# tub-rip/event_based_bos

Hardware: AMD Instinct MI355X
Metric: Mevents/sec warped+IWE at 1280x720 (higher is better)
Workload: dtype f32

## Files before the change

event_based_bos_amd/_hip.py:

```python
from __future__ import annotations

import ctypes as C
import os
from typing import Optional

import torch

_PKG_DIR = os.path.dirname(os.path.abspath(__file__))
LIB_PATH = os.path.join(_PKG_DIR, "lib", "libebos_hip.so")

EBOS_OK = 0
REF_FIRST, REF_LAST, REF_FRACTION, REF_TIMEBASE = 0, 1, 2, 3
SPLAT_BILINEAR, SPLAT_COUNT, SPLAT_POLARITY = 0, 1, 2
GAUSS_REFLECT_SCIPY, GAUSS_REFLECT_TORCH = 0, 1
PROFILE_SLAB_ACCUMULATE, PROFILE_TILED_BWD, PROFILE_SLAB_COMBINE, PROFILE_GRADMAG_FUSED = 0, 1, 2, 3
ABI_VERSION = 2
GML_NO_POLARITY, GML_EVENT_WEIGHTS = 1, 2
GML_VELOCITY = 4



_HW_QUEUES = 4
MAX_HW_QUEUES = 2

# ... 81 lines not shown
    "ebos_raw_time_range": (_I, [_P, _I, _L, _D, _P, _P, _P]),
    "ebos_raw_events_to_soa": (_I, [_P, _P, _P, _I, _P, _D, _P, _I, _D, _I, _L, _P, _P, _P, _P, _P]),
    "ebos_bin_scratch_bytes": (_Z, [_L]),
    "ebos_bin_scratch_bytes_events": (_Z, [_L, _I, _I, _I, _I]),
    "ebos_bin_events_f32": (_I, [_P, _P, _P, _P, _L, _I, _I, _I, _I, _P, _P, _P, _P, _P, _P, _P, _P, _P, _Z, _P]),
    "ebos_plan_lean_scratch_bytes": (_Z, [_L, _I, _I, _I, _I]),
    "ebos_plan_lean": (_I, [_I, _P, _P, _P, _P, _D, _L, _I, _D, _I, _I, _I, _I, _I, _P, _P, _P, _P, _L, _P, _P, _P, _Z, _P]),
    "ebos_plan_compact_f32": (_I, [_P, _P, _P, _P, _L, _I, _I, _I, _I, _P, _P, _P, _L, _P]),
    "ebos_plan_compact_frac_f32": (_I, [_P, _P, _P, _P, _L, _I, _I, _I, _I, _P, _P, _P, _P, _P, _L, _P]),
    "ebos_iwe_dense_f32": (_I, [_P, _P, _P, _P, _L, _P, _I, _I, _I, _I, _I, _P, _P]),
    "ebos_iwe_dense_tiled_f32": (_I, [_P, _P, _P, _P, _P, _L, _P, _I, _I, _I, _I, _I, _I, _I, _I, _P, _P]),
    "ebos_tiled_config": (_I, [C.POINTER(C.c_int), _I]),
    "ebos_iwe_dense_bwd_f32": (_I, [_P, _P, _P, _P, _L, _P, _I, _I, _I, _I, _I, _P, _P, _I, _I, _P, _P, _P]),
    "ebos_slab_config": (_I, [C.POINTER(C.c_int), _I]),
    "ebos_halo_auto": (_I, [_I, _D]),
    "ebos_iwe_slab_workspace_bytes": (_Z, [_I, _I, _I, _I, _I, _I, _I, _I]),
    "ebos_iwe_dense_slab_f32": (_I, [_P, _P, _P, _P, _P, _P, _P, _P, _L, _P, _I, _I, _I, _I, _I, _I, _I, _I, _P, _Z, _P, _I, _I, _P, _P, _P, _P]),
    "ebos_iwe_2dof_slab_f32": (_I, [_P, _P, _P, _P, _P, _P, _P, _P, _L, _P, _I, _I, _I, _I, _I, _I, _I, _I, _I, _P, _Z, _P, _I, _I, _P, _P, _P, _P]),
    "ebos_iwe_2dof_slab_batch_f32": (_I, [_P, _P, _P, _P, _L, _P, _I, _I, _I, _I, _I, _I, _I, _I, _I, _P, _Z, _P, _I, _I, _P, _P, _P, _P, _P]),
    "ebos_plan_parts": (_I, [_P, _I, _I, _I, _I, _I, _I, _P, _P]),
    "ebos_plan_facts": (_I, [_P, _I, _I, _I, _I, _P, _P, _P, _P]),
    "ebos_iwe_2dof_tiled_bwd_f32": (_I, [_P, _P, _P, _P, _P, _P, _P, _P, _L, _P, _I, _I, _I, _I, _I, _I, _I, _I, _P, _P, _I, _P, _P, _Z, _P]),
    "ebos_iwe_dense_tiled_bwd_f32": (_I, [_P, _P, _P, _P, _P, _P, _P, _P, _L, _P, _I, _I, _I, _I, _I, _I, _I, _P, _P, _I, _P, _P, _P, _P, _P, _P, _Z, _P, _P]),
    "ebos_variance_dense_job_f32": (_I, [_P, _P, _P, _P, _P, _P]),
    "ebos_gradient_magnitude_dense_job_f32": (_I, [_P, _P, _P, _P, _P, _P, _P, _P, _L, _P]),
    "ebos_variance_dense_job_signed_f32": (_I, [_P, _P, _P, _P, _P, _P, _P]),
    "ebos_gradient_magnitude_fused_partials": (_L, [_I, _I]),
    "ebos_gradient_magnitude_fused_f32": (_I, [_P, _I, _I, _I, _P, _P, _P, _P, _L, _P]),
    "ebos_iwe_2dof_f32": (_I, [_P, _P, _P, _P, _L, _P, _I, _I, _I, _I, _I, _P, _P]),
    "ebos_iwe_2dof_bwd_f32": (_I, [_P, _P, _P, _P, _L, _P, _I, _I, _I, _I, _I, _P, _P, _I, _P, _P]),
# ... 246 lines not shown
```

event_based_bos_amd/csrc/iwe_tile_core.h:

```cpp
#pragma once
#include <stdlib.h>

#include <atomic>
#include <type_traits>

#include <hip/hip_ext.h>

#include "common.h"
#include "patch_grid.h"
#include "blur3.h"

namespace ebos {
namespace {

constexpr float kEps = 1e-6f;
constexpr int kBlock = 1024;

#ifdef EBOS_STAMPS
__device__ unsigned long long g_stamps[4096 * 8];
__device__ unsigned long long g_stamps_bwd[4096 * 8];
#define EBOS_STAMP(k)                                                                   \
  do {                                                                                  \
    if (threadIdx.x == 0 && blockIdx.x < 4096) g_stamps[blockIdx.x * 8 + (k)] = wall_clock64(); \
  } while (0)
// ... 377 lines not shown
}
__device__ __forceinline__ float slab_load1(__amdgpu_buffer_rsrc_t r, unsigned byte) {
  return __uint_as_float(__builtin_amdgcn_raw_buffer_load_b32(r, (int)byte, 0, kAuxSc1));
}
#endif

struct ChunkQueue {
  unsigned* next;
  __device__ __forceinline__ int pull() const {
    unsigned c = 0;
    if ((threadIdx.x & (kWave - 1)) == 0) c = atomicAdd(next, 1u);
    return (int)__builtin_amdgcn_readfirstlane(c);
  }
};

#ifdef EBOS_ABL_MULTIK
#define EBOS_KLOOP for (int kk = 0; kk < EBOS_ABL_MULTIK; ++kk)
#define EBOS_KOFF(v, s) ((v) + (s) * (float)kk)
#else
#define EBOS_KLOOP
#define EBOS_KOFF(v, s) (v)
#endif

__device__ __forceinline__ int32_t chunk_group(int32_t g_first, int c, int lane) { return g_first + c * kWave + lane; }

template <int TH, int TW, int HALO, bool UNIFORM, int MODE = ACC_FX, bool GRID = false, bool DYN = false, bool PAIRS = false,
          bool HAS_W = false>
__device__ __forceinline__ unsigned long long accumulate_compact_fx(const TileRange& tr, double* s_acc, const EvPtrs& ev,
                                                          const float* __restrict__ flow, int H, int W, bool* any_spill,
                                                          const ChunkQueue& queue, const Win<TH, TW, HALO, DYN>& win,
                                                          const CRaw* pre = nullptr, float wscale = kFxScale) {
  static_assert(!HAS_W || (MODE == ACC_FX && !PAIRS && !DYN), "per-event weights: the plain fixed-point loop on the largest window");
  constexpr bool kMerge = PAIRS && MODE == ACC_FX;
  const int LH = win.LH(), LW = win.LW(), HR = win.HR(), HC = win.HC(), PT = win.P();
  const unsigned kPlane = LH * PT / 2;
  const unsigned kDummy = LH * PT;
  constexpr float kMagic = 12582912.0f;
  constexpr int kMagicBits = 0x4B400000;
  const float* __restrict__ flow1 = UNIFORM ? flow : flow + (GRID ? (int64_t)TH * TW : (int64_t)H * W);
  const float uni_u = UNIFORM ? -flow[0] : 0.0f, uni_v = UNIFORM ? -flow[1] : 0.0f;
  const unsigned base_lin = GRID ? 0u : (unsigned)(tr.ty * TH * W + tr.tx * TW);
  const unsigned uW = GRID ? (unsigned)TW : (unsigned)W;
  constexpr bool kBuf = !UNIFORM && !GRID;
  const __amdgpu_buffer_rsrc_t rsrc = __builtin_amdgcn_make_buffer_rsrc(
      reinterpret_cast<char*>(const_cast<float*>(flow)) - 4 * HC, 0, kBuf ? 2 * H * W * (int)sizeof(float) + 4 * HC : 0, 0x00020000);
  const int soff0 = (int)(base_lin * 4u), soff1 = soff0 + H * W * (int)sizeof(float);
  const unsigned uW4 = uW * 4u;
// ... 8 lines not shown
      if (kBuf) {
        u = __builtin_bit_cast(float, __builtin_amdgcn_raw_buffer_load_b32(rsrc, (int)off, soff0, 0));
        v = __builtin_bit_cast(float, __builtin_amdgcn_raw_buffer_load_b32(rsrc, (int)off, soff1, 0));
      } else {
        u = *reinterpret_cast<const float*>(flow_b0 + off);
        v = *reinterpret_cast<const float*>(flow_b1 + off);
      }
    }
  };
  bool spilled = false;
  const int32_t g_last = tr.g_last;
  const int lane = threadIdx.x & (kWave - 1), wave = threadIdx.x / kWave;
  constexpr int kWaves = kBlock / kWave;
  char* const s_bytes = reinterpret_cast<char*>(s_acc);
  unsigned long long added = 0ull;
  auto deposit = [&](const CGroupQ& cur, const float* fu, const float* fv, bool lane_live, const float4& wq4 = float4{}) {
    const float wq[4] = {wq4.x, wq4.y, wq4.z, wq4.w};
    unsigned m_byte = 0u, m00 = 0u, m01 = 0u, m10 = 0u, m11 = 0u;
#pragma unroll
    for (int e = 0; e < 4; ++e) EBOS_KLOOP {
      const float lx = -cur.dt[e] * EBOS_KOFF(fu[e], 0.37f), ly = -cur.dt[e] * EBOS_KOFF(fv[e], -0.21f);
      const float r0 = floorf(lx + kEps), c0 = floorf(ly + kEps);
      const float fr = fmaxf(lx - r0, 0.0f), fc = fmaxf(ly - c0, 0.0f);
      const int rl = (int)cur.pr[e] + HR + (int)r0;
      const int cl4 = (int)cur.pcq[e] + ((int)c0 << 2);
      const bool ok = lane_live && (fabsf(lx) + fabsf(ly) < 5.0e8f);
      const bool inside = ok && (unsigned)rl < (unsigned)(LH - 1) && (unsigned)cl4 < (unsigned)(4 * (LW - 1));
      spilled |= ok && !inside;
      if (MODE == ACC_F64) {
        const float a = 1.0f - fr, b = 1.0f - fc;
        const int cl = cl4 >> 2;
        double* cell = s_acc + (inside ? rl * PT + cl : 0);
        atomic_add(cell, (double)(inside ? a * b : 0.0f));
        atomic_add(cell + 1, (double)(inside ? a * fc : 0.0f));
        atomic_add(cell + PT, (double)(inside ? fr * b : 0.0f));
        atomic_add(cell + PT + 1, (double)(inside ? fr * fc : 0.0f));
        continue;
      }
      const float b = 1.0f - fc;
      float unit = kFxScale;
      if (HAS_W) {
        const float tu = __fmaf_rn(wq[e], wscale, kMagic);
        unit = tu - kMagic;
// ... 80 lines not shown
  float fu[4], fv[4];
#pragma unroll
  for (int e = 0; e < 4; ++e) fetch(cur.pr[e], cur.pcq[e], fu[e], fv[e]);
  while (chunk_group(tr.g_first, c_cur, 0) <= g_last) {
    const int32_t grp = chunk_group(tr.g_first, c_cur, lane);
    float gu[4], gv[4];
#pragma unroll
    for (int e = 0; e < 4; ++e) fetch(nxt.pr[e], nxt.pcq[e], gu[e], gv[e]);
    const int c_nn = queue.pull();
    CGroupQ nn;
    load_cgroup_q(nn, chunk_group(tr.g_first, c_nn, lane), tr, ev, hc4);
    float4 w_nn = float4{};
    if (HAS_W) w_nn = weights_of(c_nn);
    const bool lane_live = grp <= g_last;
    deposit(cur, fu, fv, lane_live, w_cur);
    cur = nxt;
    nxt = nn;
    w_cur = w_nxt;
    w_nxt = w_nn;
    c_cur = c_nxt;
    c_nxt = c_nn;
#pragma unroll
    for (int e = 0; e < 4; ++e) {
      fu[e] = gu[e];
      fv[e] = gv[e];
    }
  }
  }
  if (any_spill) *any_spill = spilled;
  return added;
}

enum Pass { PASS_MAIN = 0, PASS_SPILL = 1 };

template <int TH, int TW, int HALO, bool HAS_W, int MODE, int PASS, int FMT, bool UNIFORM, bool GRID = false, bool DYN = false,
          bool PAIRS = false, bool FRAC = false>
__device__ __forceinline__ unsigned long long accumulate_slice(const TileRange& tr, double* s_acc, const EvPtrs& ev,
                                                     const float* __restrict__ flow, int H, int W, int pad_h, int pad_w,
                                                     float* spill, bool* any_spill, const ChunkQueue& queue,
                                                     const Win<TH, TW, HALO, DYN>& win, const CRaw* pre = nullptr,
                                                     float wscale = kFxScale) {
  const int LH = win.LH(), LW = win.LW(), PT = win.P();
  unsigned long long* s_fx = reinterpret_cast<unsigned long long*>(s_acc);
  const int h = H + 2 * pad_h, w = W + 2 * pad_w;
  const int tr0 = tr.ty * TH, tc0 = tr.tx * TW;
  const int oy = tr0 - win.HR(), ox = tc0 - win.HC();
  const float* __restrict__ flow1 = UNIFORM ? flow : flow + (GRID ? (int64_t)TH * TW : (int64_t)H * W);
  const float uni_u = UNIFORM ? -flow[0] : 0.0f, uni_v = UNIFORM ? -flow[1] : 0.0f;
  const int fl_r0 = GRID ? tr0 : 0, fl_c0 = GRID ? tc0 : 0, fl_w = GRID ? TW : W;
  unsigned long long added = 0;
  bool spilled = false;
  if (tr.g_first > tr.g_last) return 0;
  if (FMT == FMT_COMPACT && PASS == PASS_MAIN && !HAS_W && !FRAC)
    return accumulate_compact_fx<TH, TW, HALO, UNIFORM, MODE, GRID, DYN, PAIRS>(tr, s_acc, ev, flow, H, W, any_spill, queue, win, pre);
  if constexpr (FMT == FMT_COMPACT && PASS == PASS_MAIN && HAS_W && !FRAC && MODE == ACC_FX && !DYN && !PAIRS)
    return accumulate_compact_fx<TH, TW, HALO, UNIFORM, ACC_FX, GRID, false, false, true>(tr, s_acc, ev, flow, H, W, any_spill, queue, win,
                                                                                       nullptr, wscale);
  const int32_t g_last = tr.g_last;
  int32_t grp = tr.g_first + threadIdx.x;
  Group cur, nxt;
  load_group<FMT, HAS_W, TH, TW>(cur, grp, tr, ev, tr0, tc0);
  load_group<FMT, HAS_W, TH, TW>(nxt, grp + kBlock, tr, ev, tr0, tc0);
  float fu[4], fv[4];
#pragma unroll
  for (int e = 0; e < 4; ++e) {
    const int lin = (cur.rs[e] - fl_r0) * fl_w + (cur.cs[e] - fl_c0);
    fu[e] = UNIFORM ? uni_u : flow[lin];
    fv[e] = UNIFORM ? uni_v : flow1[lin];
  }
// ... 194 lines not shown
      return;
    }
    const float wr = blur3_axis_weight(R, h, lo, bk);
    const float e[4] = {v.x, v.y, v.z, v.w};
#pragma unroll
    for (int k = 0; k < 4; ++k)
      if (C + k >= 0 && C + k < w) acc_b += (double)(wr * blur3_axis_weight(C + k, w, lo, bk)) * (double)e[k];
  }
  __device__ __forceinline__ double total() const {
    if (bk.k0 == 0.0f) return acc;
    const float wi = blur3_axis_weight(lo + 2, max(h, 2 * lo + 5), lo, bk);
    return (double)(wi * wi) * acc + acc_b;
  }
};

template <int TH, int TW, int HALO, bool HAS_W, int MODE, int FMT, bool UNIFORM, bool GRID, bool DYN, bool ZERO, bool FRAC = false,
          typename Hook, typename Own>
__device__ __forceinline__ void tile_body(const TileRange& tr, const Win<TH, TW, HALO, DYN>& win, const float* flow, double* s_acc,
                                          TileShared& sh, const EvPtrs& ev, int H, int W, int tiles_x, int pad_h, int pad_w,
                                          float* __restrict__ slabs, float* spill, unsigned* __restrict__ spill_epoch, unsigned epoch,
                                          unsigned* __restrict__ halo_tab, const CRaw* pre, Hook&& after_loop, Own& own) {
  constexpr int kLHmax = TH + 2 * HALO, kLWmax = TW + 2 * HALO;
  constexpr int kCells = acc_cells<TH, TW, HALO, DYN>();
  const ChunkQueue queue{&sh.next};
  const int LH = win.LH(), LW = win.LW(), PT = win.P();
  if (DYN && halo_tab != nullptr && threadIdx.x == 0) halo_tab[tr.ty * tiles_x + tr.tx] = win_pack(win.hr, win.hc);
  EBOS_STAMP(1);

  bool spilled = false;
  unsigned long long added;
  constexpr bool kCanPair = DYN && FMT == FMT_COMPACT && !HAS_W && MODE == ACC_FX && !FRAC;
  const int32_t n_ev = tr.end - tr.beg;
  if (kCanPair && n_ev >= 4 * TH * TW && ((win.HR() <= 16 && win.HC() <= 16) || n_ev >= 24 * TH * TW))
    added = accumulate_slice<TH, TW, HALO, HAS_W, MODE, PASS_MAIN, FMT, UNIFORM, GRID, DYN, kCanPair>(
        tr, s_acc, ev, flow, H, W, pad_h, pad_w, spill, &spilled, queue, win, nullptr);
  else
    added = accumulate_slice<TH, TW, HALO, HAS_W, MODE, PASS_MAIN, FMT, UNIFORM, GRID, DYN, false, FRAC>(
        tr, s_acc, ev, flow, H, W, pad_h, pad_w, spill, &spilled, queue, win, pre, HAS_W ? sh.wscale : kFxScale);
  after_loop();
  constexpr bool kLeanLoop = FMT == FMT_COMPACT && !HAS_W && !FRAC;
  if (kLeanLoop && threadIdx.x == 0 && tr.g_first <= tr.g_last)
    added += (unsigned long long)(min(tr.end, tr.beg + 4 * (tr.g_last - tr.g_first + 1)) - tr.beg) << kFxShift;
  if (spilled) sh.flag[1] = 1;
  EBOS_STAMP(2);
  __syncthreads();
  EBOS_STAMP(3);
  if (sh.flag[1] && spill_epoch != nullptr && threadIdx.x == 0) *spill_epoch = epoch;
  if (sh.flag[1] && spill != nullptr)
    added -= accumulate_slice<TH, TW, HALO, HAS_W, MODE, PASS_SPILL, FMT, UNIFORM, GRID, DYN, false, FRAC>(tr, s_acc, ev, flow, H, W, pad_h,
                                                                                                           pad_w, spill, nullptr, queue, win);

  float4* out = reinterpret_cast<float4*>(slabs + (int64_t)tr.slab * (kLHmax * kLWmax));
#ifndef EBOS_PLAIN_SLABS
  const __amdgpu_buffer_rsrc_t out_rsrc = slab_rsrc(reinterpret_cast<const float*>(out), (unsigned)(kLHmax * kLWmax * sizeof(float)));
#define EBOS_SLAB_STORE(i, v) slab_store4(out_rsrc, (unsigned)(i) * 16u, (v))
#else
#define EBOS_SLAB_STORE(i, v) out[i] = (v)
#endif
  bool f64_flush = (MODE == ACC_F64);
  if (MODE == ACC_FX) {
    uint2* pa = reinterpret_cast<uint2*>(s_acc);
    uint2* pb = pa + LH * PT / 2;
    unsigned long long decoded = 0;
    const float kInv = HAS_W ? sh.wdec : (float)kFxInv;
    auto decode_quad = [&](int r, int j, int slab_quad) {
      const int wrow = r * (PT / 2);
      const uint2 a0 = pa[wrow + 2 * j], a1 = pa[wrow + 2 * j + 1];
      const uint2 b0 = pb[wrow + 2 * j], b1 = pb[wrow + 2 * j + 1];
      const unsigned bmh = j > 0 ? pb[wrow + 2 * j - 1].y : 0u;
      if (ZERO) {
        const uint2 z = make_uint2(0u, 0u);
        pa[wrow + 2 * j] = z, pa[wrow + 2 * j + 1] = z;
        pb[wrow + 2 * j] = z, pb[wrow + 2 * j + 1] = z;
      }
      decoded += ((unsigned long long)a0.x + a0.y) + ((unsigned long long)a1.x + a1.y) + ((unsigned long long)b0.x + b0.y) +
                 ((unsigned long long)b1.x + b1.y);
      const float4 v4 = make_float4(((float)a0.x + (float)bmh) * kInv, ((float)a0.y + (float)b0.x) * kInv,
                                    ((float)a1.x + (float)b0.y) * kInv, ((float)a1.y + (float)b1.x) * kInv);
      EBOS_SLAB_STORE(slab_quad, v4);
      own(r, j, v4);
    };
    if (ZERO) {
      const int q = LW / 4, rpi = kWave / q;
      const int lane = threadIdx.x & (kWave - 1), wave = threadIdx.x / kWave;
      int sub = 0, j = lane;
      while (j >= q) j -= q, ++sub;
      const bool act = sub < rpi;
      for (int r0 = wave * rpi; r0 < LH; r0 += (kBlock / kWave) * rpi) {
        const int r = r0 + sub;
        if (act && r < LH) decode_quad(r, j, r * q + j);
      }
      for (int i = threadIdx.x; i < PT / 2 + 2; i += kBlock) reinterpret_cast<unsigned long long*>(s_acc)[LH * PT + i] = 0ull;
    } else {
      const int q = LW / 4;
      const float inv_q = 1.0f / (float)q;
      for (int i = threadIdx.x; i < LH * q; i += kBlock) {
        const int r = DYN ? (int)(((float)i + 0.5f) * inv_q) : i / q;
        decode_quad(r, i - r * q, i);
      }
    }
#ifdef EBOS_ABL_MULTIK
    const unsigned long long diff = 0ull * wave_sum(added - decoded);
#else
    const unsigned long long diff = wave_sum(added - decoded);
#endif
    if ((threadIdx.x & (kWave - 1)) == 0 && diff != 0ull) atomicAdd(&sh.chk, diff);
    __syncthreads();
    if (sh.chk != 0ull) {
      for (int i = threadIdx.x; i < kCells; i += kBlock) s_acc[i] = 0.0;
      if (threadIdx.x == 0) sh.next = 2 * (kBlock / kWave);
      __syncthreads();
      accumulate_slice<TH, TW, HALO, HAS_W, ACC_F64, PASS_MAIN, FMT, UNIFORM, GRID, DYN, false, FRAC>(tr, s_acc, ev, flow, H, W, pad_h, pad_w,
                                                                                                      spill, nullptr, queue, win);
      __syncthreads();
      f64_flush = true;
    }
  }
  if (f64_flush) {
    const int q = LW / 4;
    const float inv_q = 1.0f / (float)q;
    own.reset();
    for (int i = threadIdx.x; i < LH * q; i += kBlock) {
      const int r = DYN ? (int)(((float)i + 0.5f) * inv_q) : i / q;
      double* p = &s_acc[r * PT + 4 * (i - r * q)];
      const float4 v4 = make_float4((float)p[0], (float)p[1], (float)p[2], (float)p[3]);
      EBOS_SLAB_STORE(i, v4);
      own(r, i - r * q, v4);
      if (ZERO) p[0] = p[1] = p[2] = p[3] = 0.0;
    }
    if (ZERO)
      for (int i = threadIdx.x; i < PT / 2 + 2; i += kBlock) s_acc[LH * PT + i] = 0.0;
  }
  EBOS_STAMP(4);
}


template <int TH, int TW, int HALO, bool HAS_W, int MODE, int FMT, bool UNIFORM, bool GRID = false, bool DYN = false, bool ZERO = false,
          bool FRAC = false>
__device__ __forceinline__ void accumulate_tile(const EvPtrs& ev, const int32_t* __restrict__ key_offsets,
                                                const float* __restrict__ flow_arg, int H, int W, int tiles_x, int splits, int pad_h,
                                                int pad_w, float* __restrict__ slabs, float* spill, const GridSrc& gs,
                                                unsigned* __restrict__ spill_epoch, unsigned epoch, float dt_bound = 0.0f,
                                                unsigned* __restrict__ halo_tab = nullptr) {
  constexpr int kLWmax = TW + 2 * HALO;
  constexpr int kCells = acc_cells<TH, TW, HALO, DYN>();
  static_assert(kLWmax % 4 == 0, "slab rows are written 4 cells at a time");
  static_assert(!DYN || (FMT == FMT_COMPACT && !HAS_W), "run-time windows: the lean loop only");
  extern __shared__ double s_acc[];
  __shared__ TileShared sh;
  EBOS_STAMP(0);
  static_assert(kCells % 2 == 0, "LDS image is cleared 16 bytes per lane");
  constexpr bool kBoundFromFlow = DYN && !GRID && !UNIFORM;
  if (!GRID && !kBoundFromFlow)
// ... 9 lines not shown
#ifndef EBOS_PLAIN_SLABS
    const __amdgpu_buffer_rsrc_t zr = slab_rsrc(reinterpret_cast<const float*>(out0), (unsigned)((TH + 2 * HALO) * kLWmax * sizeof(float)));
    for (int i = threadIdx.x; i < n4; i += kBlock) slab_store4(zr, (unsigned)i * 16u, make_float4(0.f, 0.f, 0.f, 0.f));
#else
    for (int i = threadIdx.x; i < n4; i += kBlock) out0[i] = make_float4(0.f, 0.f, 0.f, 0.f);
#endif
    return;
  }
  constexpr bool kLeanPre = FMT == FMT_COMPACT && !HAS_W && MODE == ACC_FX && !FRAC;
  CRaw pre[2];
  if (kLeanPre) {
    const int lane = threadIdx.x & (kWave - 1), wave = threadIdx.x / kWave;
    pre[0] = load_craw(tr.g_first + wave * kWave + lane, tr, ev);
    pre[1] = load_craw(tr.g_first + (wave + kBlock / kWave) * kWave + lane, tr, ev);
  }
  float mu = 0.0f, mv = 0.0f;
  if (kBoundFromFlow) {
    tile_flow_absmax<TH, TW>(flow_arg, H, W, tr.ty * TH, tr.tx * TW, mu, mv);
    for (int i = threadIdx.x; i < kCells / 2; i += kBlock) reinterpret_cast<double2*>(s_acc)[i] = make_double2(0.0, 0.0);
  }

  const float* flow = flow_arg;
  float* s_flow = reinterpret_cast<float*>(s_acc + kCells);
  Lerp* s_lerp = reinterpret_cast<Lerp*>(s_flow + 2 * TH * TW);
  TileGrid tg{};
  if (GRID) {
    tg = tile_grid_begin<TH, TW, 0>(flow_arg, gs, tr.ty * TH, tr.tx * TW, H, W, s_lerp);
    for (int i = threadIdx.x; i < kCells / 2; i += kBlock) reinterpret_cast<double2*>(s_acc)[i] = make_double2(0.0, 0.0);
  }
  if (threadIdx.x < 2) sh.flag[threadIdx.x] = 0;
// ... 49 lines not shown
    flow = s_flow;
  }
  __syncthreads();
  const Win<TH, TW, HALO, DYN> win = tile_bound_read<TH, TW, HALO, DYN>(sh.bound, dt_bound);
  NoOwn no_own;
  if constexpr (HAS_W && MODE == ACC_FX) {
    if (sh.flag[0]) {
      __syncthreads();
      if (threadIdx.x == 0) sh.flag[0] = 0;
      __syncthreads();
      tile_body<TH, TW, HALO, HAS_W, ACC_F64, FMT, UNIFORM, GRID, DYN, ZERO>(tr, win, flow, s_acc, sh, ev, H, W, tiles_x, pad_h, pad_w, slabs,
                                                                            spill, spill_epoch, epoch, halo_tab, nullptr, NoHook{}, no_own);
      return;
    }
  }
  tile_body<TH, TW, HALO, HAS_W, MODE, FMT, UNIFORM, GRID, DYN, ZERO, FRAC>(tr, win, flow, s_acc, sh, ev, H, W, tiles_x, pad_h, pad_w, slabs,
                                                                           spill, spill_epoch, epoch, halo_tab, kLeanPre ? pre : nullptr,
                                                                           NoHook{}, no_own);
}

template <int TH, int TW, int HALO, bool HAS_W, int MODE, int FMT, bool UNIFORM, bool GRID = false, bool DYN = false, bool FRAC = false>
__global__ void __launch_bounds__(kBlock)
iwe_slab_accumulate_kernel(EvPtrs ev, const int32_t* __restrict__ key_offsets, const float* __restrict__ flow_arg, int H, int W,
                           int tiles_x, int splits, int pad_h, int pad_w, float* __restrict__ slabs, float* spill, GridSrc gs,
                           unsigned* __restrict__ spill_epoch, unsigned epoch, float dt_bound, unsigned* __restrict__ halo_tab) {
  accumulate_tile<TH, TW, HALO, HAS_W, MODE, FMT, UNIFORM, GRID, DYN, false, FRAC>(ev, key_offsets, flow_arg, H, W, tiles_x, splits, pad_h,
                                                                                  pad_w, slabs, spill, gs, spill_epoch, epoch, dt_bound,
                                                                                  halo_tab);
}

struct FwdWindow {
  EvPtrs ev;
  const int32_t* key_offsets;
  const float* flow;
  float* slabs;
  float* spill;
  unsigned* spill_epoch;
  unsigned* halo_tab;
  double* partials;
  float* iwe;
  float* out_var;
  double* moments;
};
// ... 1527 lines not shown
```

event_based_bos_amd/csrc/iwe_tiled.hip:

```cpp
#include "iwe_tiled_launch.h"

namespace ebos {

unsigned next_spill_epoch() {
  static std::atomic<unsigned> counter{0};
  unsigned e = counter.fetch_add(1, std::memory_order_relaxed) + 1;
  if (e == 0) e = counter.fetch_add(1, std::memory_order_relaxed) + 1;
  return e;
}

namespace {

inline hipEvent_t next_order_event() {
  constexpr int kRing = 64, kMaxDevices = 64;
  struct Ring {
    hipEvent_t ev[kRing];
    std::atomic<unsigned> created{0}, cursor{0};
    std::atomic_flag lock = ATOMIC_FLAG_INIT;
  };
  static Ring rings[kMaxDevices];
  int dev = 0;
  if (hipGetDevice(&dev) != hipSuccess || dev < 0 || dev >= kMaxDevices) return nullptr;
  Ring& r = rings[dev];
  if (r.created.load(std::memory_order_acquire) == 0) {
// ... 53 lines not shown
  else if (tile_h == 64 && tile_w == 64 && halo == 16) { rc = CALL(64, 64, 16); } \
  else if (tile_h == 45 && tile_w == 80 && halo == 16) { rc = CALL(45, 80, 16); } \
  else if (tile_h == 32 && tile_w == 32 && halo == 16) { rc = CALL(32, 32, 16); } \
  else if (tile_h == 32 && tile_w == 32 && halo == 8) { rc = CALL(32, 32, 8); }

extern "C" {

int ebos_slab_config(int* out, int cap) {
  using namespace ebos;
  for (int i = 0; i < kNumSlabConfigs && i < cap && out != nullptr; ++i) {
    out[3 * i] = kSlabConfigs[i].th;
    out[3 * i + 1] = kSlabConfigs[i].tw;
    out[3 * i + 2] = kSlabConfigs[i].halo;
  }
  return kNumSlabConfigs;
}

int ebos_halo_auto(int max_halo, double dt_bound) {
  if (max_halo <= 0 || max_halo > 255 || !(dt_bound >= 0.0) || dt_bound > 4096.0) return max_halo;
  int q = (int)(dt_bound * 64.0);
  if ((double)q < dt_bound * 64.0) ++q;
  return EBOS_HALO_AUTO(max_halo, q < 1 ? 1 : q);
}

int ebos_iwe_slab_partials(int H, int W, int tile_h, int tile_w, int halo_arg, int splits, int pad_h, int pad_w, int omit_boundary,
                           size_t* offset_bytes, int64_t* n_partials, int64_t* n_pixels) {
  using namespace ebos;
  const int halo = decode_halo(halo_arg).halo;
  EBOS_REQUIRE(offset_bytes && n_partials && n_pixels, "ebos_iwe_slab_partials: NULL output");
  EBOS_REQUIRE(H > 0 && W > 0 && tile_h > 0 && tile_w > 0 && halo >= 0 && splits >= 0 && pad_h >= 0 && pad_w >= 0,
// ... 639 lines not shown
```

event_based_bos_amd/csrc/iwe_tiled_launch.h:

```cpp
#pragma once
#include "iwe_tile_core.h"

namespace ebos {

unsigned next_spill_epoch();
int order_after(hipStream_t later, hipStream_t earlier, const char* what);

struct SlabOps {
  int th, tw, halo;
  int (*fwd)(const EvPtrs& ev, const int32_t* key_offsets, const float* flow, bool uniform, int H, int W, int splits, int pad_h, int pad_w,
             char* ws, float* iwe, int want_var, int omit, float* out_var, double* moments, int acc_mode, hipStream_t s,
             const GridSrc* grid_src, const HaloArg& ha);
  int (*fwd_batch)(const FwdBatch& b, int n, int H, int W, int splits, int pad_h, int pad_w, int want_var, int omit, hipStream_t s,
                   hipStream_t s_tail, const GridSrc* grid_src, const HaloArg& ha, bool uniform);
  int (*bwd)(const EvPtrs& ev, const int32_t* key_offsets, const float* flow, bool uniform, int H, int W, int pad_h, int pad_w,
             const float* g_image, const float* affine, int g_lo, float* d_flow, float* d_weight, double* partials,
             const double* var_moments, const float* upstream, const float* addend, float* part_out, hipStream_t s,
             const GridSrc* grid_src, int adaptive, float s_norm, float s_tv, double* reg_partials, MomentsIn mj, const HaloArg& ha,
             bool finalize_uniform);
};
const SlabOps* slab_ops(int th, int tw, int halo);

#ifdef EBOS_SLAB_OPS_UNIT
namespace {
// ... 20 lines not shown
  void (*ka)(EvPtrs, const int32_t*, const float*, int, int, int, int, int, int, float*, float*, GridSrc, unsigned*, unsigned, float,
             unsigned*);
  const bool compact = ev.cpix != nullptr;
  const bool dyn = ha.dyn && compact && ev.w == nullptr && acc_mode == ACC_FX;
  if (dyn) lds = (size_t)acc_cells<TH, TW, HALO, true>() * sizeof(double);
  GridSrc gs{};
#define EBOS_PICK(HW, MD)                                                                                              \
  (uniform ? (compact ? iwe_slab_accumulate_kernel<TH, TW, HALO, HW, MD, FMT_COMPACT, true>                            \
                      : iwe_slab_accumulate_kernel<TH, TW, HALO, HW, MD, FMT_XY, true>)                                 \
           : (compact ? iwe_slab_accumulate_kernel<TH, TW, HALO, HW, MD, FMT_COMPACT, false>                           \
                      : iwe_slab_accumulate_kernel<TH, TW, HALO, HW, MD, FMT_XY, false>))
  if (ev.w) ka = acc_mode == ACC_F64 ? EBOS_PICK(true, ACC_F64) : EBOS_PICK(true, ACC_FX);
  else if (acc_mode == ACC_F64) ka = EBOS_PICK(false, ACC_F64);
  else ka = EBOS_PICK(false, ACC_FX);
#undef EBOS_PICK
  if (dyn)
    ka = uniform ? iwe_slab_accumulate_kernel<TH, TW, HALO, false, ACC_FX, FMT_COMPACT, true, false, true>
                 : iwe_slab_accumulate_kernel<TH, TW, HALO, false, ACC_FX, FMT_COMPACT, false, false, true>;
  if (compact && ev.cfx != nullptr && grid_src == nullptr) {
    if (!uniform || ev.w != nullptr || acc_mode != ACC_FX) {
      set_error("ebos_iwe_*_slab: fractions per compact slot (cfx / cfy) go with the 2-DoF model or the patch grid, unit weights");
      return EBOS_ERR_UNSUPPORTED;
    }
    ka = dyn ? iwe_slab_accumulate_kernel<TH, TW, HALO, false, ACC_FX, FMT_COMPACT, true, false, true, true>
             : iwe_slab_accumulate_kernel<TH, TW, HALO, false, ACC_FX, FMT_COMPACT, true, false, false, true>;
  }
  if (grid_src != nullptr) {
    if constexpr (grid_fwd_fits<TH, TW, HALO>()) {
      if (!compact || uniform) {
        set_error("ebos_iwe_patch_slab: needs the compact plan format and unit weights");
// ... 197 lines not shown
```

include/ebos_hip.h:

```cpp
#ifndef EBOS_HIP_H
#define EBOS_HIP_H

#include <stddef.h>
#include <stdint.h>

#ifdef __cplusplus
extern "C" {
#endif

#define EBOS_ABI_VERSION 2

typedef void* ebos_stream_t;

typedef enum ebos_status {
  EBOS_OK = 0,
  EBOS_ERR_INVALID_ARG = -1,
  EBOS_ERR_LAUNCH = -2,
  EBOS_ERR_UNSUPPORTED = -3,
  EBOS_ERR_SCRATCH = -4
} ebos_status;

typedef enum ebos_reftime_mode {
  EBOS_REF_FIRST = 0,
  EBOS_REF_LAST = 1,
// ... 110 lines not shown
                       ebos_stream_t stream);
int ebos_iwe_dense_tiled_f32(const float* xs, const float* ys, const float* dts, const float* weight,
                             const int32_t* key_offsets, int64_t n, const float* flow, int H, int W,
                             int tile_h, int tile_w, int halo, int splits, int pad_h, int pad_w,
                             float* iwe, ebos_stream_t stream);
int ebos_tiled_config(int* out, int cap);

int ebos_iwe_dense_bwd_f32(const float* x, const float* y, const float* dt, const float* weight, int64_t n,
                           const float* flow, int H, int W, int row_stride, int pad_h, int pad_w,
                           const float* g_image, const float* affine, int g_lo, int sorted, float* d_flow,
                           float* d_weight, ebos_stream_t stream);

#define EBOS_HALO_AUTO(max_halo, dt_bound_q64) (-((int)(max_halo) + 256 * (int)(dt_bound_q64)))
int ebos_halo_auto(int max_halo, double dt_bound);
int ebos_slab_config(int* out, int cap);
size_t ebos_iwe_slab_workspace_bytes(int H, int W, int tile_h, int tile_w, int halo, int splits, int pad_h,
                                     int pad_w);
int ebos_iwe_slab_partials(int H, int W, int tile_h, int tile_w, int halo, int splits, int pad_h, int pad_w,
                           int omit_boundary, size_t* offset_bytes, int64_t* n_partials, int64_t* n_pixels);
int ebos_iwe_dense_slab_f32(const float* xs, const float* ys, const float* dts, const float* weight,
                            const int32_t* grp_offsets, const uint16_t* cpix, const float* cdt,
                            const int32_t* key_offsets, int64_t n, const float* flow, int H, int W, int tile_h,
                            int tile_w, int halo, int splits, int pad_h, int pad_w, void* workspace,
                            size_t workspace_bytes, float* iwe, int want_variance, int omit_boundary,
                            float* out_variance, double* moments, const int32_t* part_table,
                            ebos_stream_t stream);
typedef struct ebos_dense_job {
  const float *xs, *ys, *dts;
  const int32_t* grp_offsets;
  const uint16_t* cpix;
// ... 401 lines not shown
```

Baseline: 368,700.

## Flush finished slab rows early while waves still accumulate events

Adds an early-flush mode to the 45x80/halo-32 fixed-point slab accumulate kernel. Each wave publishes its chunk progress in shared memory. Waves that run out of work then decode and store the accumulator rows that no pending event can still touch, claimed in blocks via CAS, so the slab write overlaps the tail of accumulation. It falls back to a full re-decode if any event lands above the row window, and it adds shared-memory polling, atomics and store waits. The mode is on by default and can be turned off with an env var or an API call.

```diff
diff --git a/event_based_bos_amd/_hip.py b/event_based_bos_amd/_hip.py
--- a/event_based_bos_amd/_hip.py
+++ b/event_based_bos_amd/_hip.py
@@ -119,6 +119,7 @@
     "ebos_iwe_dense_bwd_f32": (_I, [_P, _P, _P, _P, _L, _P, _I, _I, _I, _I, _I, _P, _P, _I, _I, _P, _P, _P]),
     "ebos_slab_config": (_I, [C.POINTER(C.c_int), _I]),
     "ebos_halo_auto": (_I, [_I, _D]),
+    "ebos_set_early_flush": (_I, [_I]),
     "ebos_iwe_slab_workspace_bytes": (_Z, [_I, _I, _I, _I, _I, _I, _I, _I]),
     "ebos_iwe_dense_slab_f32": (_I, [_P, _P, _P, _P, _P, _P, _P, _P, _L, _P, _I, _I, _I, _I, _I, _I, _I, _I, _P, _Z, _P, _I, _I, _P, _P, _P, _P]),
     "ebos_iwe_2dof_slab_f32": (_I, [_P, _P, _P, _P, _P, _P, _P, _P, _L, _P, _I, _I, _I, _I, _I, _I, _I, _I, _I, _P, _Z, _P, _I, _I, _P, _P, _P, _P]),
diff --git a/event_based_bos_amd/csrc/iwe_tile_core.h b/event_based_bos_amd/csrc/iwe_tile_core.h
--- a/event_based_bos_amd/csrc/iwe_tile_core.h
+++ b/event_based_bos_amd/csrc/iwe_tile_core.h
@@ -415,6 +415,14 @@
   }
 };
 
+constexpr int kFlushQuads = 128, kFlushClaim = 2;
+struct EarlyShared {
+  unsigned cur[kBlock / kWave];
+  unsigned block;
+  int back;
+};
+__device__ __forceinline__ void wait_own_stores() { __builtin_amdgcn_s_waitcnt(0x0F70); }
+
 #ifdef EBOS_ABL_MULTIK
 #define EBOS_KLOOP for (int kk = 0; kk < EBOS_ABL_MULTIK; ++kk)
 #define EBOS_KOFF(v, s) ((v) + (s) * (float)kk)
@@ -426,12 +434,14 @@
 __device__ __forceinline__ int32_t chunk_group(int32_t g_first, int c, int lane) { return g_first + c * kWave + lane; }
 
 template <int TH, int TW, int HALO, bool UNIFORM, int MODE = ACC_FX, bool GRID = false, bool DYN = false, bool PAIRS = false,
-          bool HAS_W = false>
+          bool HAS_W = false, bool EARLY = false>
 __device__ __forceinline__ unsigned long long accumulate_compact_fx(const TileRange& tr, double* s_acc, const EvPtrs& ev,
                                                           const float* __restrict__ flow, int H, int W, bool* any_spill,
                                                           const ChunkQueue& queue, const Win<TH, TW, HALO, DYN>& win,
-                                                          const CRaw* pre = nullptr, float wscale = kFxScale) {
+                                                          const CRaw* pre = nullptr, float wscale = kFxScale,
+                                                          EarlyShared* es = nullptr) {
   static_assert(!HAS_W || (MODE == ACC_FX && !PAIRS && !DYN), "per-event weights: the plain fixed-point loop on the largest window");
+  static_assert(!EARLY || (MODE == ACC_FX && !PAIRS && !HAS_W), "early flush: the plain fixed-point loop with unit weights");
   constexpr bool kMerge = PAIRS && MODE == ACC_FX;
   const int LH = win.LH(), LW = win.LW(), HR = win.HR(), HC = win.HC(), PT = win.P();
   const unsigned kPlane = LH * PT / 2;
@@ -470,6 +480,7 @@
   constexpr int kWaves = kBlock / kWave;
   char* const s_bytes = reinterpret_cast<char*>(s_acc);
   unsigned long long added = 0ull;
+  float r_min = 0.0f;
   auto deposit = [&](const CGroupQ& cur, const float* fu, const float* fv, bool lane_live, const float4& wq4 = float4{}) {
     const float wq[4] = {wq4.x, wq4.y, wq4.z, wq4.w};
     unsigned m_byte = 0u, m00 = 0u, m01 = 0u, m10 = 0u, m11 = 0u;
@@ -483,6 +494,7 @@
       const bool ok = lane_live && (fabsf(lx) + fabsf(ly) < 5.0e8f);
       const bool inside = ok && (unsigned)rl < (unsigned)(LH - 1) && (unsigned)cl4 < (unsigned)(4 * (LW - 1));
       spilled |= ok && !inside;
+      if constexpr (EARLY) r_min = fminf(r_min, r0);
       if (MODE == ACC_F64) {
         const float a = 1.0f - fr, b = 1.0f - fc;
         const int cl = cl4 >> 2;
@@ -593,6 +605,10 @@
     if (HAS_W) w_nn = weights_of(c_nn);
     const bool lane_live = grp <= g_last;
     deposit(cur, fu, fv, lane_live, w_cur);
+    if constexpr (EARLY)
+      if (lane == 0)
+        __hip_atomic_store(&es->cur[wave], ((unsigned)c_nxt << 1) | (chunk_group(tr.g_first, c_nn, 0) <= g_last ? 0u : 1u), __ATOMIC_RELAXED,
+                           __HIP_MEMORY_SCOPE_WORKGROUP);
     cur = nxt;
     nxt = nn;
     w_cur = w_nxt;
@@ -607,18 +623,21 @@
   }
   }
   if (any_spill) *any_spill = spilled;
+  if constexpr (EARLY)
+    if (r_min < -(float)HR) es->back = 1;
   return added;
 }
 
 enum Pass { PASS_MAIN = 0, PASS_SPILL = 1 };
 
 template <int TH, int TW, int HALO, bool HAS_W, int MODE, int PASS, int FMT, bool UNIFORM, bool GRID = false, bool DYN = false,
-          bool PAIRS = false, bool FRAC = false>
+          bool PAIRS = false, bool FRAC = false, bool EARLY = false>
 __device__ __forceinline__ unsigned long long accumulate_slice(const TileRange& tr, double* s_acc, const EvPtrs& ev,
                                                      const float* __restrict__ flow, int H, int W, int pad_h, int pad_w,
                                                      float* spill, bool* any_spill, const ChunkQueue& queue,
                                                      const Win<TH, TW, HALO, DYN>& win, const CRaw* pre = nullptr,
-                                                     float wscale = kFxScale) {
+                                                     float wscale = kFxScale, EarlyShared* es = nullptr) {
+  static_assert(!EARLY || (FMT == FMT_COMPACT && PASS == PASS_MAIN && !HAS_W && !FRAC), "early flush: the lean hot loop only");
   const int LH = win.LH(), LW = win.LW(), PT = win.P();
   unsigned long long* s_fx = reinterpret_cast<unsigned long long*>(s_acc);
   const int h = H + 2 * pad_h, w = W + 2 * pad_w;
@@ -631,7 +650,8 @@
   bool spilled = false;
   if (tr.g_first > tr.g_last) return 0;
   if (FMT == FMT_COMPACT && PASS == PASS_MAIN && !HAS_W && !FRAC)
-    return accumulate_compact_fx<TH, TW, HALO, UNIFORM, MODE, GRID, DYN, PAIRS>(tr, s_acc, ev, flow, H, W, any_spill, queue, win, pre);
+    return accumulate_compact_fx<TH, TW, HALO, UNIFORM, MODE, GRID, DYN, PAIRS, false, EARLY>(tr, s_acc, ev, flow, H, W, any_spill, queue, win,
+                                                                                              pre, kFxScale, es);
   if constexpr (FMT == FMT_COMPACT && PASS == PASS_MAIN && HAS_W && !FRAC && MODE == ACC_FX && !DYN && !PAIRS)
     return accumulate_compact_fx<TH, TW, HALO, UNIFORM, ACC_FX, GRID, false, false, true>(tr, s_acc, ev, flow, H, W, any_spill, queue, win,
                                                                                        nullptr, wscale);
@@ -856,12 +876,44 @@
   }
 };
 
+#ifndef EBOS_PLAIN_SLABS
+#define EBOS_SLAB_ARG out_rsrc,
+#define EBOS_SLAB_PARAM __amdgpu_buffer_rsrc_t out_rsrc,
+#define EBOS_SLAB_STORE(i, v) slab_store4(out_rsrc, (unsigned)(i) * 16u, (v))
+#else
+#define EBOS_SLAB_ARG
+#define EBOS_SLAB_PARAM
+#define EBOS_SLAB_STORE(i, v) out[i] = (v)
+#endif
+template <bool ZERO, typename Own>
+__device__ __forceinline__ void decode_quad_fx(uint2* pa, uint2* pb, int PT, float kInv, float4* out, EBOS_SLAB_PARAM int r, int j,
+                                               int slab_quad, unsigned long long& decoded, Own& own) {
+  const int wrow = r * (PT / 2);
+  const uint2 a0 = pa[wrow + 2 * j], a1 = pa[wrow + 2 * j + 1];
+  const uint2 b0 = pb[wrow + 2 * j], b1 = pb[wrow + 2 * j + 1];
+  const unsigned bmh = j > 0 ? pb[wrow + 2 * j - 1].y : 0u;
+  if (ZERO) {
+    const uint2 z = make_uint2(0u, 0u);
+    pa[wrow + 2 * j] = z, pa[wrow + 2 * j + 1] = z;
+    pb[wrow + 2 * j] = z, pb[wrow + 2 * j + 1] = z;
+  }
+  decoded += ((unsigned long long)a0.x + a0.y) + ((unsigned long long)a1.x + a1.y) + ((unsigned long long)b0.x + b0.y) +
+             ((unsigned long long)b1.x + b1.y);
+  const float4 v4 = make_float4(((float)a0.x + (float)bmh) * kInv, ((float)a0.y + (float)b0.x) * kInv,
+                                ((float)a1.x + (float)b0.y) * kInv, ((float)a1.y + (float)b1.x) * kInv);
+  EBOS_SLAB_STORE(slab_quad, v4);
+  own(r, j, v4);
+}
+
 template <int TH, int TW, int HALO, bool HAS_W, int MODE, int FMT, bool UNIFORM, bool GRID, bool DYN, bool ZERO, bool FRAC = false,
-          typename Hook, typename Own>
+          bool EARLY = false, typename Hook, typename Own>
 __device__ __forceinline__ void tile_body(const TileRange& tr, const Win<TH, TW, HALO, DYN>& win, const float* flow, double* s_acc,
                                           TileShared& sh, const EvPtrs& ev, int H, int W, int tiles_x, int pad_h, int pad_w,
                                           float* __restrict__ slabs, float* spill, unsigned* __restrict__ spill_epoch, unsigned epoch,
-                                          unsigned* __restrict__ halo_tab, const CRaw* pre, Hook&& after_loop, Own& own) {
+                                          unsigned* __restrict__ halo_tab, const CRaw* pre, Hook&& after_loop, Own& own,
+                                          EarlyShared* es = nullptr, int32_t row_first = 0) {
+  static_assert(!EARLY || (MODE == ACC_FX && FMT == FMT_COMPACT && !HAS_W && !FRAC && !DYN && !ZERO && TH < kWave),
+                "early flush: the lean fixed-point loop on a built window, one work item per workgroup");
   constexpr int kLHmax = TH + 2 * HALO, kLWmax = TW + 2 * HALO;
   constexpr int kCells = acc_cells<TH, TW, HALO, DYN>();
   const ChunkQueue queue{&sh.next};
@@ -871,14 +923,50 @@
 
   bool spilled = false;
   unsigned long long added;
+  unsigned long long decoded_early = 0;
   constexpr bool kCanPair = DYN && FMT == FMT_COMPACT && !HAS_W && MODE == ACC_FX && !FRAC;
   const int32_t n_ev = tr.end - tr.beg;
   if (kCanPair && n_ev >= 4 * TH * TW && ((win.HR() <= 16 && win.HC() <= 16) || n_ev >= 24 * TH * TW))
     added = accumulate_slice<TH, TW, HALO, HAS_W, MODE, PASS_MAIN, FMT, UNIFORM, GRID, DYN, kCanPair>(
         tr, s_acc, ev, flow, H, W, pad_h, pad_w, spill, &spilled, queue, win, nullptr);
   else
-    added = accumulate_slice<TH, TW, HALO, HAS_W, MODE, PASS_MAIN, FMT, UNIFORM, GRID, DYN, false, FRAC>(
-        tr, s_acc, ev, flow, H, W, pad_h, pad_w, spill, &spilled, queue, win, pre, HAS_W ? sh.wscale : kFxScale);
+    added = accumulate_slice<TH, TW, HALO, HAS_W, MODE, PASS_MAIN, FMT, UNIFORM, GRID, DYN, false, FRAC, EARLY>(
+        tr, s_acc, ev, flow, H, W, pad_h, pad_w, spill, &spilled, queue, win, pre, HAS_W ? sh.wscale : kFxScale, es);
+  if constexpr (EARLY) {
+    const int lane = threadIdx.x & (kWave - 1);
+    const int q = LW / 4;
+    float4* out = reinterpret_cast<float4*>(slabs + (int64_t)tr.slab * (kLHmax * kLWmax));
+#ifndef EBOS_PLAIN_SLABS
+    const __amdgpu_buffer_rsrc_t out_rsrc = slab_rsrc(reinterpret_cast<const float*>(out), (unsigned)(kLHmax * kLWmax * sizeof(float)));
+#endif
+    uint2* pa = reinterpret_cast<uint2*>(s_acc);
+    uint2* pb = pa + LH * PT / 2;
+    const int n_chunks = (tr.g_last - tr.g_first + kWave) / kWave;
+    while (tr.g_first <= tr.g_last) {
+      const unsigned c = __hip_atomic_load(&es->cur[lane & (kBlock / kWave - 1)], __ATOMIC_RELAXED, __HIP_MEMORY_SCOPE_WORKGROUP);
+      const unsigned b = __builtin_amdgcn_readfirstlane(__hip_atomic_load(&es->block, __ATOMIC_RELAXED, __HIP_MEMORY_SCOPE_WORKGROUP));
+      unsigned f = __builtin_amdgcn_readlane(c, 0) >> 1;
+#pragma unroll
+      for (int k = 1; k < kBlock / kWave; ++k) f = min(f, (unsigned)__builtin_amdgcn_readlane(c, k) >> 1);
+      if (__builtin_amdgcn_ballot_w64(lane < kBlock / kWave && (c & 1u) == 0u && (int)(c >> 1) < n_chunks) == 0ull) break;
+      const int32_t limit = tr.beg + 4 * kWave * (int32_t)f;
+      const bool below = lane <= TH && row_first <= limit;
+      const int rows = __builtin_popcountll(__builtin_amdgcn_ballot_w64(below)) - 1;
+      const int avail = rows * q / kFlushQuads - (int)b;
+      if (avail <= 0) break;
+      const int take = min(avail, kFlushClaim);
+      unsigned won = 0u;
+      if (lane == 0) won = atomicCAS(&es->block, b, b + (unsigned)take) == b ? 1u : 0u;
+      if (__builtin_amdgcn_readfirstlane(won) == 0u) continue;
+      __builtin_amdgcn_fence(__ATOMIC_ACQUIRE, "wavefront");
+#pragma unroll
+      for (int k = 0; k < kFlushClaim * kFlushQuads / kWave; ++k) {
+        const int i = (int)b * kFlushQuads + k * kWave + lane;
+        const int r = i / q;
+        if (k * kWave < take * kFlushQuads) decode_quad_fx<false>(pa, pb, PT, (float)kFxInv, out, EBOS_SLAB_ARG r, i - r * q, i, decoded_early, own);
+      }
+    }
+  }
   after_loop();
   constexpr bool kLeanLoop = FMT == FMT_COMPACT && !HAS_W && !FRAC;
   if (kLeanLoop && threadIdx.x == 0 && tr.g_first <= tr.g_last)
@@ -895,9 +983,6 @@
   float4* out = reinterpret_cast<float4*>(slabs + (int64_t)tr.slab * (kLHmax * kLWmax));
 #ifndef EBOS_PLAIN_SLABS
   const __amdgpu_buffer_rsrc_t out_rsrc = slab_rsrc(reinterpret_cast<const float*>(out), (unsigned)(kLHmax * kLWmax * sizeof(float)));
-#define EBOS_SLAB_STORE(i, v) slab_store4(out_rsrc, (unsigned)(i) * 16u, (v))
-#else
-#define EBOS_SLAB_STORE(i, v) out[i] = (v)
 #endif
   bool f64_flush = (MODE == ACC_F64);
   if (MODE == ACC_FX) {
@@ -906,22 +991,23 @@
     unsigned long long decoded = 0;
     const float kInv = HAS_W ? sh.wdec : (float)kFxInv;
     auto decode_quad = [&](int r, int j, int slab_quad) {
-      const int wrow = r * (PT / 2);
-      const uint2 a0 = pa[wrow + 2 * j], a1 = pa[wrow + 2 * j + 1];
-      const uint2 b0 = pb[wrow + 2 * j], b1 = pb[wrow + 2 * j + 1];
-      const unsigned bmh = j > 0 ? pb[wrow + 2 * j - 1].y : 0u;
-      if (ZERO) {
-        const uint2 z = make_uint2(0u, 0u);
-        pa[wrow + 2 * j] = z, pa[wrow + 2 * j + 1] = z;
-        pb[wrow + 2 * j] = z, pb[wrow + 2 * j + 1] = z;
-      }
-      decoded += ((unsigned long long)a0.x + a0.y) + ((unsigned long long)a1.x + a1.y) + ((unsigned long long)b0.x + b0.y) +
-                 ((unsigned long long)b1.x + b1.y);
-      const float4 v4 = make_float4(((float)a0.x + (float)bmh) * kInv, ((float)a0.y + (float)b0.x) * kInv,
-                                    ((float)a1.x + (float)b0.y) * kInv, ((float)a1.y + (float)b1.x) * kInv);
-      EBOS_SLAB_STORE(slab_quad, v4);
-      own(r, j, v4);
+      decode_quad_fx<ZERO>(pa, pb, PT, kInv, out, EBOS_SLAB_ARG r, j, slab_quad, decoded, own);
     };
+    int first_quad = 0;
+    if constexpr (EARLY) {
+      first_quad = (int)es->block * kFlushQuads;
+      decoded = decoded_early;
+      if (es->back) {
+        wait_own_stores();
+        __syncthreads();
+        first_quad = 0;
+        decoded = 0;
+        own.reset();
+      }
+#ifdef EBOS_STAMPS
+      if (threadIdx.x == 0 && blockIdx.x < 4096) g_stamps[blockIdx.x * 8 + 7] = (unsigned long long)(es->block * kFlushQuads / (LW / 4));
+#endif
+    }
     if (ZERO) {
       const int q = LW / 4, rpi = kWave / q;
       const int lane = threadIdx.x & (kWave - 1), wave = threadIdx.x / kWave;
@@ -936,7 +1022,7 @@
     } else {
       const int q = LW / 4;
       const float inv_q = 1.0f / (float)q;
-      for (int i = threadIdx.x; i < LH * q; i += kBlock) {
+      for (int i = first_quad + threadIdx.x; i < LH * q; i += kBlock) {
         const int r = DYN ? (int)(((float)i + 0.5f) * inv_q) : i / q;
         decode_quad(r, i - r * q, i);
       }
@@ -951,6 +1037,7 @@
     if (sh.chk != 0ull) {
       for (int i = threadIdx.x; i < kCells; i += kBlock) s_acc[i] = 0.0;
       if (threadIdx.x == 0) sh.next = 2 * (kBlock / kWave);
+      if constexpr (EARLY) wait_own_stores();
       __syncthreads();
       accumulate_slice<TH, TW, HALO, HAS_W, ACC_F64, PASS_MAIN, FMT, UNIFORM, GRID, DYN, false, FRAC>(tr, s_acc, ev, flow, H, W, pad_h, pad_w,
                                                                                                       spill, nullptr, queue, win);
@@ -978,7 +1065,7 @@
 
 
 template <int TH, int TW, int HALO, bool HAS_W, int MODE, int FMT, bool UNIFORM, bool GRID = false, bool DYN = false, bool ZERO = false,
-          bool FRAC = false>
+          bool FRAC = false, bool EARLY = false>
 __device__ __forceinline__ void accumulate_tile(const EvPtrs& ev, const int32_t* __restrict__ key_offsets,
                                                 const float* __restrict__ flow_arg, int H, int W, int tiles_x, int splits, int pad_h,
                                                 int pad_w, float* __restrict__ slabs, float* spill, const GridSrc& gs,
@@ -1018,6 +1105,16 @@
     pre[0] = load_craw(tr.g_first + wave * kWave + lane, tr, ev);
     pre[1] = load_craw(tr.g_first + (wave + kBlock / kWave) * kWave + lane, tr, ev);
   }
+  EarlyShared* es = nullptr;
+  int32_t row_first = 0;
+  if constexpr (EARLY) {
+    __shared__ EarlyShared s_early;
+    es = &s_early;
+    if (threadIdx.x < kBlock / kWave)
+      es->cur[threadIdx.x] = (threadIdx.x << 1) | (chunk_group(tr.g_first, (int)threadIdx.x + kBlock / kWave, 0) <= tr.g_last ? 0u : 1u);
+    if (threadIdx.x == 0) es->block = 0u, es->back = 0;
+    row_first = key_offsets[(int64_t)(tr.ty * tiles_x + tr.tx) * (TH * TW) + min((int)(threadIdx.x & (kWave - 1)), TH) * TW];
+  }
   float mu = 0.0f, mv = 0.0f;
   if (kBoundFromFlow) {
     tile_flow_absmax<TH, TW>(flow_arg, H, W, tr.ty * TH, tr.tx * TW, mu, mv);
@@ -1097,19 +1194,20 @@
       return;
     }
   }
-  tile_body<TH, TW, HALO, HAS_W, MODE, FMT, UNIFORM, GRID, DYN, ZERO, FRAC>(tr, win, flow, s_acc, sh, ev, H, W, tiles_x, pad_h, pad_w, slabs,
-                                                                           spill, spill_epoch, epoch, halo_tab, kLeanPre ? pre : nullptr,
-                                                                           NoHook{}, no_own);
-}
-
-template <int TH, int TW, int HALO, bool HAS_W, int MODE, int FMT, bool UNIFORM, bool GRID = false, bool DYN = false, bool FRAC = false>
+  tile_body<TH, TW, HALO, HAS_W, MODE, FMT, UNIFORM, GRID, DYN, ZERO, FRAC, EARLY>(tr, win, flow, s_acc, sh, ev, H, W, tiles_x, pad_h, pad_w,
+                                                                                  slabs, spill, spill_epoch, epoch, halo_tab,
+                                                                                  kLeanPre ? pre : nullptr, NoHook{}, no_own, es, row_first);
+}
+
+template <int TH, int TW, int HALO, bool HAS_W, int MODE, int FMT, bool UNIFORM, bool GRID = false, bool DYN = false, bool FRAC = false,
+          bool EARLY = false>
 __global__ void __launch_bounds__(kBlock)
 iwe_slab_accumulate_kernel(EvPtrs ev, const int32_t* __restrict__ key_offsets, const float* __restrict__ flow_arg, int H, int W,
                            int tiles_x, int splits, int pad_h, int pad_w, float* __restrict__ slabs, float* spill, GridSrc gs,
                            unsigned* __restrict__ spill_epoch, unsigned epoch, float dt_bound, unsigned* __restrict__ halo_tab) {
-  accumulate_tile<TH, TW, HALO, HAS_W, MODE, FMT, UNIFORM, GRID, DYN, false, FRAC>(ev, key_offsets, flow_arg, H, W, tiles_x, splits, pad_h,
-                                                                                  pad_w, slabs, spill, gs, spill_epoch, epoch, dt_bound,
-                                                                                  halo_tab);
+  accumulate_tile<TH, TW, HALO, HAS_W, MODE, FMT, UNIFORM, GRID, DYN, false, FRAC, EARLY>(ev, key_offsets, flow_arg, H, W, tiles_x, splits,
+                                                                                         pad_h, pad_w, slabs, spill, gs, spill_epoch, epoch,
+                                                                                         dt_bound, halo_tab);
 }
 
 struct FwdWindow {
diff --git a/event_based_bos_amd/csrc/iwe_tiled.hip b/event_based_bos_amd/csrc/iwe_tiled.hip
--- a/event_based_bos_amd/csrc/iwe_tiled.hip
+++ b/event_based_bos_amd/csrc/iwe_tiled.hip
@@ -7,6 +7,17 @@
   unsigned e = counter.fetch_add(1, std::memory_order_relaxed) + 1;
   if (e == 0) e = counter.fetch_add(1, std::memory_order_relaxed) + 1;
   return e;
+}
+
+static std::atomic<int> g_early_flush{-1};
+bool early_flush_enabled() {
+  int v = g_early_flush.load(std::memory_order_relaxed);
+  if (v < 0) {
+    const char* e = getenv("EBOS_NO_EARLY_FLUSH");
+    v = (e && e[0] != '\0' && e[0] != '0') ? 0 : 1;
+    g_early_flush.store(v, std::memory_order_relaxed);
+  }
+  return v != 0;
 }
 
 namespace {
@@ -91,6 +102,12 @@
     out[3 * i + 2] = kSlabConfigs[i].halo;
   }
   return kNumSlabConfigs;
+}
+
+int ebos_set_early_flush(int on) {
+  const int before = ebos::early_flush_enabled() ? 1 : 0;
+  ebos::g_early_flush.store(on ? 1 : 0, std::memory_order_relaxed);
+  return before;
 }
 
 int ebos_halo_auto(int max_halo, double dt_bound) {
diff --git a/event_based_bos_amd/csrc/iwe_tiled_launch.h b/event_based_bos_amd/csrc/iwe_tiled_launch.h
--- a/event_based_bos_amd/csrc/iwe_tiled_launch.h
+++ b/event_based_bos_amd/csrc/iwe_tiled_launch.h
@@ -5,6 +5,7 @@
 
 unsigned next_spill_epoch();
 int order_after(hipStream_t later, hipStream_t earlier, const char* what);
+bool early_flush_enabled();
 
 struct SlabOps {
   int th, tw, halo;
@@ -58,6 +59,9 @@
   else if (acc_mode == ACC_F64) ka = EBOS_PICK(false, ACC_F64);
   else ka = EBOS_PICK(false, ACC_FX);
 #undef EBOS_PICK
+  if constexpr (TH == 45 && TW == 80 && HALO == 32)
+    if (ka == iwe_slab_accumulate_kernel<TH, TW, HALO, false, ACC_FX, FMT_COMPACT, false> && early_flush_enabled())
+      ka = iwe_slab_accumulate_kernel<TH, TW, HALO, false, ACC_FX, FMT_COMPACT, false, false, false, false, true>;
   if (dyn)
     ka = uniform ? iwe_slab_accumulate_kernel<TH, TW, HALO, false, ACC_FX, FMT_COMPACT, true, false, true>
                  : iwe_slab_accumulate_kernel<TH, TW, HALO, false, ACC_FX, FMT_COMPACT, false, false, true>;
diff --git a/include/ebos_hip.h b/include/ebos_hip.h
--- a/include/ebos_hip.h
+++ b/include/ebos_hip.h
@@ -148,6 +148,7 @@
 #define EBOS_HALO_AUTO(max_halo, dt_bound_q64) (-((int)(max_halo) + 256 * (int)(dt_bound_q64)))
 int ebos_halo_auto(int max_halo, double dt_bound);
 int ebos_slab_config(int* out, int cap);
+int ebos_set_early_flush(int on);
 size_t ebos_iwe_slab_workspace_bytes(int H, int W, int tile_h, int tile_w, int halo, int splits, int pad_h,
                                      int pad_w);
 int ebos_iwe_slab_partials(int H, int W, int tile_h, int tile_w, int halo, int splits, int pad_h, int pad_w,
```

After: 349,400. 5.2% lower.
